# Clemapfel/kmer_index

Hardware: AMD Instinct MI355X
Metric: M queries/sec, DNA4 k=10 exact-match batch search, 1e8-bp text (higher is better)
Workload: dtype u32/u64

## Files before the change

kmer_index_amd/csrc/kmx_capi.hip:

```cpp
#include <hip/hip_runtime.h>

#include <algorithm>
#include <atomic>
#include <cstddef>
#include <cstdio>
#include <cstdlib>
#include <cstring>
#include <functional>
#include <memory>
#include <mutex>
#include <string>
#include <system_error>
#include <thread>
#include <utility>
#include <vector>

#include "kmx_approx.h"
#include "kmx_host.h"
#include "kmx_kernels.h"
#include "kmx_vote.h"

namespace {

thread_local std::string g_err;
// ... 305 lines not shown

void release_idle(ResultPool& pool)
{
    std::vector<kmx_result*> idle;
    { std::lock_guard<std::mutex> lock(pool.mu); idle.swap(pool.idle); }
    for (kmx_result* r : idle) { r->release(); delete r; }
}

kmx_result* take_result(kmx_index* ix)
{
    kmx_result* r = nullptr;
    {
        std::lock_guard<std::mutex> lock(ix->pool->mu);
        if (!ix->pool->idle.empty()) { r = ix->pool->idle.back(); ix->pool->idle.pop_back(); }
    }
    if (!r) r = new kmx_result();
    r->pool = ix->pool;
    return r;
}

template <typename F>
void timed(kmx_index* ix, int id, hipStream_t s, F&& launch)
{
    if (!ix->stats.enabled) { launch(); return; }
    std::lock_guard<std::mutex> lock(ix->stats.mu);
    hipEvent_t a = ix->stats.get(), b = ix->stats.get();
    (void)hipEventRecord(a, s);
    launch();
    (void)hipEventRecord(b, s);
    ix->stats.pending.push_back({id, a, b});
}

template <typename T>
kmx_status upload(kmx_index* ix, const T* host, size_t count, const T** dev_out)
{
    void* p = nullptr;
    size_t bytes = std::max<size_t>(count * sizeof(T), 16) + 16;
    HIP_TRY(hipMalloc(&p, bytes));
    ix->allocs.push_back(p);
    ix->device_bytes += bytes;
    if (count) HIP_TRY(hipMemcpy(p, host, count * sizeof(T), hipMemcpyHostToDevice));
    *dev_out = static_cast<const T*>(p);
    return KMX_OK;
}

struct DeviceScratch {
    std::vector<void*> ptrs;
    ~DeviceScratch() { for (void* p : ptrs) (void)hipFree(p); }
    template <typename T> hipError_t get(T** out, size_t count)
    {
        void* p = nullptr;
        hipError_t e = hipMalloc(&p, count * sizeof(T) + 64);
        if (e == hipSuccess) { ptrs.push_back(p); *out = static_cast<T*>(p); }
        return e;
    }
};

kmx_status check_device()
{
    int count = 0;
    hipError_t e = hipGetDeviceCount(&count);
    if (e != hipSuccess || count <= 0)
        return fail(KMX_ERR_NO_DEVICE, "no HIP device visible: the kmx engine has no CPU search path");
    return KMX_OK;
}

}

static uint32_t cell_shift_for(uint32_t table_kind, uint64_t n_keys, uint64_t npos, uint64_t region, const kmx_options& o)
{
    if (table_kind != KMX_TABLE_DENSE || o.no_aligned_copy || region > npos) return 0;
    if (const char* e = getenv("KMX_CELLS")) { if (!atoi(e)) return 0; }
    const double c = double(npos) / double(n_keys);
    uint32_t shift = c <= 3.5 ? 3u : c <= 10.5 ? 4u : c <= 24.0 ? 5u : 0u;
    if (const char* e = getenv("KMX_CELL_SHIFT")) { const int v = atoi(e); if (v >= 3 && v <= 5) shift = uint32_t(v); }
    if (!shift) return 0;
    if ((n_keys << shift) > 8 * npos) return 0;
    return shift;
}
static inline uint64_t up32_elems(uint64_t v) { return (v + 31) & ~uint64_t(31); }

static hipError_t publish_headers(kmx_index* ix)
{
    hipError_t e = hipMemcpy(ix->d_index, &ix->h_header, sizeof(KmxIndexDev), hipMemcpyHostToDevice);
    if (e == hipSuccess && ix->d_index_fast) {
        KmxIndexDev hf = ix->h_header;
        if (ix->d_plan_fast) hf.plan = ix->d_plan_fast;
        e = hipMemcpy(ix->d_index_fast, &hf, sizeof hf, hipMemcpyHostToDevice);
    }
    return e;
}
static inline const KmxIndexDev* header_for(const kmx_index* ix, uint32_t flags)
{
    static const bool ref_plan_only = getenv("KMX_REFERENCE_PLAN") != nullptr;
    return ((flags & (KMX_SEARCH_KEEP_MASKS | KMX_SEARCH_REFERENCE_PLAN)) || !ix->d_index_fast || ref_plan_only) ? ix->d_index : ix->d_index_fast;
}

static kmx_status install_images_impl(std::vector<kmx::ElemImage>& images, const uint8_t* tail_kmax, uint64_t n, uint32_t sigma,
                                 uint32_t range, int device, const kmx_options& o, kmx_index** out, void* prebuilt_arena,
                                 uint64_t prebuilt_arena_elems = 0)
{
    auto* ix = new kmx_index();
    ix->device = device;
    ix->n = n;
    ix->sigma = sigma;
    ix->range = range;
    const uint32_t n_ks = uint32_t(images.size());
    uint32_t kmax = 0;
    for (auto& im : images) { ix->ks.push_back(im.k); kmax = std::max(kmax, im.k); }
    kmx_status st = KMX_OK;
    auto bail = [&](kmx_status s) { std::string keep = g_err; kmx_index_free(ix); g_err = keep; return s; };
    for (auto& im : images) {
        if (im.d_offs_prebuilt) ix->allocs.push_back(const_cast<uint32_t*>(im.d_offs_prebuilt));
        if (im.d_atab_prebuilt) ix->allocs.push_back(const_cast<uint32_t*>(im.d_atab_prebuilt));
        if (im.d_ukeys_prebuilt) ix->allocs.push_back(const_cast<uint64_t*>(im.d_ukeys_prebuilt));
        if (im.d_slots_prebuilt) ix->allocs.push_back(const_cast<KmxSlot*>(im.d_slots_prebuilt));
    }

    KmxIndexDev h{};
    h.n = n; h.sigma = sigma; h.n_ks = n_ks; h.kmax = kmax; h.range = range;
    for (uint32_t j = 0; j < 64; ++j) {
        unsigned __int128 v = 1;
        for (uint32_t t = 0; t < j; ++t) { v *= sigma; if (v > ~uint64_t(0)) { v = ~uint64_t(0); break; } }
        h.pw[j] = uint64_t(v);
    }
    uint64_t arena_elems = 0;
    for (auto& im : images) {
        if (!im.region) im.region = im.npos;
        if (im.region > im.npos) arena_elems = (arena_elems + 31) & ~uint64_t(31);
        arena_elems += im.region;
    }
    std::vector<uint32_t> cell_shift(n_ks, 0);
    std::vector<uint64_t> cell_base(n_ks, 0);
    for (uint32_t i = 0; i < n_ks; ++i) {
        const auto& im = images[i];
        cell_shift[i] = cell_shift_for(im.table_kind, im.n_keys, im.npos, im.region, o);
        if (cell_shift[i] && (up32_elems(arena_elems) + (im.n_keys << cell_shift[i]) + 65536) * 4 >= (uint64_t(1) << 32)) cell_shift[i] = 0;
        if (!cell_shift[i]) continue;
        arena_elems = up32_elems(arena_elems);
        cell_base[i] = arena_elems;
        arena_elems += im.n_keys << cell_shift[i];
    }
    if (prebuilt_arena && prebuilt_arena_elems < arena_elems) {
        fail(KMX_ERR_INVALID_ARGUMENT, "internal: the prebuilt arena is smaller than the index layout");
        return bail(KMX_ERR_INVALID_ARGUMENT);
    }
    {
        void* p = prebuilt_arena;
        if (!p) {
            hipError_t e = hipMalloc(&p, arena_elems * 4 + KMX_ARENA_PAD);
            if (e != hipSuccess) { fail(KMX_ERR_OUT_OF_MEMORY, std::string("arena: ") + hipGetErrorString(e)); return bail(KMX_ERR_OUT_OF_MEMORY); }
        }
        ix->allocs.push_back(p);
        ix->device_bytes += arena_elems * 4;
        {
            hipError_t e = hipMemset(static_cast<unsigned char*>(p) + arena_elems * 4, 0xFF, KMX_ARENA_PAD);
            if (e != hipSuccess) { fail(KMX_ERR_HIP, std::string("arena padding: ") + hipGetErrorString(e)); return bail(KMX_ERR_HIP); }
        }
        h.arena = static_cast<const uint32_t*>(p);
        ix->d_arena = h.arena;
    }
    h.arena_elems = arena_elems;
    ix->rec32 = (arena_elems + 65536) * 4 < (uint64_t(1) << 32);
    if (const char* f64 = getenv("KMX_FORCE_REC64")) { if (atoi(f64)) ix->rec32 = false; }
    if (const char* fvs = getenv("KMX_FILL_VARIANT")) {
        int e = atoi(fvs);
// ... 2355 lines not shown
```

kmer_index_amd/csrc/kmx_kernels.hip:

```cpp
#include <hip/hip_runtime.h>
#include <stdint.h>

#include <algorithm>
#include <atomic>
#include <type_traits>

#include "kmx_kernels.h"

#define KMX_BLOCK 256
#define KMX_WAVE 64
#define KMX_PSORT_PAIR_CAP 512
#ifndef KMX_PSORT_MULTIWAY_RUNS
#define KMX_PSORT_MULTIWAY_RUNS 4
#endif
#define KMX_PM_WAVE_EMAX (((KMX_PSORT_CAP + (KMX_WAVE - KMX_PSORT_MAX_RUNS / 2) - 1) / (KMX_WAVE - KMX_PSORT_MAX_RUNS / 2)) | 1)
#define KMX_PM_WAVE_PAD (KMX_PSORT_MAX_RUNS + KMX_PM_WAVE_EMAX + 5)
#define KMX_PM_TILE 4096
#define KMX_STAGE_CAP 1024
#define KMX_VGROUP 16
#define KMX_VGROUPS (KMX_WAVE / KMX_VGROUP)
#define KMX_VSLICES (64 / KMX_VGROUP)
#define KMX_VSTAGE (1024 / KMX_VGROUPS)
#define KMX_VCH 8

// ... 328 lines not shown
                            key = extra.src;
                            p1 = (uint64_t(extra_delta) << 32) | extra.cnt | (P - 1 + (rest ? 1 : 0) > 1 ? KMX_P1_MORE : 0);
                            if (!(flags & KMX_SEARCH_KEEP_MASKS) && stitch_goes_big(first.cnt, extra.cnt)) p1 |= KMX_P1_BIG;
                            if (track) {
                                const uint32_t lo = alive ? uint32_t(__ffs(int(alive))) - 1u : 0u, len = uint32_t(__popc(alive));
                                if ((alive >> lo) == (1u << len) - 1u) {
                                    resolved = true;
                                    src = first.src + lo;
                                    cnt = len;
                                }
                            }
                        }
                    }
                }
            }
        } else {
            uint64_t mm = m;
            bool all = true;
            Run r{0, 0}, extra{0, 0};
            uint32_t extra_delta = 0;
            const uint32_t nparts = pe.nparts;
            for (uint32_t j = 0; j < nparts && all && ranks_ok; ++j) {
                const KmxPlanEntry e = load_plan_chain(ix, mm);
                const KmxElemDev* el = &elems_s[e.elem];
                const uint32_t k = el->k;
                mm -= k;
                uint64_t h;
                ranks_ok = rank_hash(qr + mm, k, sigma, h, qend);
                if (!ranks_ok) break;
                r = probe(el, h);
                if (j == 0) {
                    extra = r; extra_delta = uint32_t(mm);
                    track = !(flags & KMX_SEARCH_KEEP_MASKS) && nparts > 1 && sparse_buckets(el) && r.cnt != 0 && r.cnt <= KMX_VRESOLVE;
                    if (track) {
                        alive = 0;
#pragma unroll
                        for (uint32_t i = 0; i < KMX_VRESOLVE; ++i) {
                            const uint32_t a = ar[r.src + (i < r.cnt ? i : 0u)];
                            cand[i] = a - uint32_t(mm);
                            alive |= uint32_t(i < r.cnt && a >= uint32_t(mm)) << i;
                        }
                    }
                } else if (track && r.cnt) {
                    follow(r, uint32_t(mm));
                }
                all = r.cnt != 0;
            }
            if (all && ranks_ok) {
                if (nparts == 1) { kind = KMX_KIND_EXACT; src = r.src; cnt = r.cnt; }
                else {
                    kind = KMX_KIND_STITCH; src = r.src; c0 = r.cnt;
                    key = extra.src;
                    p1 = (uint64_t(extra_delta) << 32) | extra.cnt | (nparts > 2 ? KMX_P1_MORE : 0);
                    if (!(flags & KMX_SEARCH_KEEP_MASKS) && stitch_goes_big(r.cnt, extra.cnt)) p1 |= KMX_P1_BIG;
                    if (track) {
                        uint32_t fmask = 0;
                        for (uint32_t t = 0; t < r.cnt; ++t) {
                            const uint32_t b = ar[r.src + t];
#pragma unroll
                            for (uint32_t i = 0; i < KMX_VRESOLVE; ++i) fmask |= uint32_t(((alive >> i) & 1u) && cand[i] == b) << t;
                        }
                        const uint32_t lo = fmask ? uint32_t(__ffs(int(fmask))) - 1u : 0u, len = uint32_t(__popc(fmask));
                        if ((fmask >> lo) == (1u << len) - 1u) {
                            resolved = true;
                            src = r.src + lo;
                            cnt = len;
                        }
                    }
                }
            }
        }
        if (!ranks_ok) { status = KMX_Q_BAD_RANK; kind = KMX_KIND_NONE; cnt = 0; }
    }
    o.src = src; o.aux = aux; o.key = key; o.p1 = p1; o.cnt = cnt; o.c0 = c0; o.kind = kind; o.status = status; o.resolved = resolved;
}

struct BlockCounters {
    unsigned int n_long, base_long;
    unsigned int n_stitch, n_stitch_tiny, n_stitch_short, n_resolved, n_prefix, n_prefix_big, n_prefix_merge, n_prefix_mid, n_prefix_plain, n_error, n_none, n_more;
    unsigned long long words, pelems, hits;
    unsigned int max_runs;
    unsigned int base_stitch, base_stitch_tiny, base_stitch_short, base_prefix, base_prefix_big;
    unsigned long long base_words;
    unsigned int max_fan_exp;
    unsigned int small_keys;
};

template <bool SMALL>
__device__ __forceinline__ bool hash16(const u32x4_a1& w, uint32_t len, uint32_t sigma, uint64_t& h)
{
    uint64_t lo = uint64_t(w[0]) | (uint64_t(w[1]) << 32), hi = uint64_t(w[2]) | (uint64_t(w[3]) << 32);
    {
        const uint32_t sh = (16u - len) * 8u;
        const uint32_t s6 = sh & 63u;
        const uint64_t carry = s6 ? lo >> (64u - s6) : 0;
        const uint64_t hi1 = (hi << s6) | carry, lo1 = lo << s6;
        hi = sh >= 128u ? 0 : sh >= 64u ? lo1 : hi1;
        lo = sh >= 64u ? 0 : lo1;
    }
    const uint32_t wd[4] = {uint32_t(lo), uint32_t(lo >> 32), uint32_t(hi), uint32_t(hi >> 32)};
    uint32_t top = 0;
    if (SMALL) {
        uint32_t acc = 0;
#pragma unroll
        for (uint32_t j = 0; j < 16; ++j) {
            const uint32_t r = (wd[j >> 2] >> (8 * (j & 3))) & 0xFFu;
            top = max(top, r);
            acc = __umul24(acc, sigma) + r;
        }
        h = acc;
    } else {
        uint64_t acc = 0;
#pragma unroll
        for (uint32_t j = 0; j < 16; ++j) {
            const uint32_t r = (wd[j >> 2] >> (8 * (j & 3))) & 0xFFu;
            top = max(top, r);
            acc = acc * sigma + r;
        }
        h = acc;
    }
    return top < sigma;
}
__device__ __forceinline__ const char* probe_first_addr(const KmxElemDev* el, uint64_t h)
{
    if (el->table_kind == KMX_TABLE_DENSE)
        return el->cnt8 ? reinterpret_cast<const char*>(el->cnt8 + (h & ~uint64_t(15)))
                        : reinterpret_cast<const char*>((el->atab ? el->atab : el->offs) + h);
    return reinterpret_cast<const char*>(el->slots + slot_hash_dev(h, el->log2cap));
}
__device__ __forceinline__ Run probe_finish(const KmxElemDev* el, uint64_t h, const u32x4_a1& pr)
{
    Run r{0, 0};
    if (el->table_kind == KMX_TABLE_DENSE) {
        if (el->cnt8) {
            const uint32_t b = uint32_t(h) & 15u;
            const uint32_t wsel = (b >> 2) == 0 ? pr[0] : (b >> 2) == 1 ? pr[1] : (b >> 2) == 2 ? pr[2] : pr[3];
            const uint32_t c = (wsel >> ((b & 3u) * 8u)) & 0xFFu;
            if (c != 255u) { r.src = el->cell_base + (h << el->cell_shift); r.cnt = c; }
            else {
                const KMX_GLOBAL uint32_t* offs = as_global(el->offs);
                const uint32_t a = offs[h], e = offs[h + 1];
                r.src = el->arena_base + a; r.cnt = e - a;
            }
        }
        else if (el->atab) { r.src = el->arena_base + (pr[0] & ~31u); r.cnt = atab_count(pr[0], pr[1]); }
        else { r.src = el->arena_base + pr[0]; r.cnt = pr[1] - pr[0]; }
        return r;
    }
    const KMX_GLOBAL KmxSlot* slots = as_global(el->slots);
    const uint64_t mask = (uint64_t(1) << el->log2cap) - 1;
    uint64_t s = slot_hash_dev(h, el->log2cap);
    uint64_t key = uint64_t(pr[0]) | (uint64_t(pr[1]) << 32);
    uint32_t off = pr[2], c = pr[3];
    while (c != 0 && key != h) {
        s = (s + 1) & mask;
        const u64x2 raw = *(const KMX_GLOBAL u64x2*)(slots + s);
        key = raw.x; off = uint32_t(raw.y); c = uint32_t(raw.y >> 32);
    }
    if (c) { r.src = el->arena_base + off; r.cnt = c; }
    return r;
}

#define KMX_PLAN_LDS 256

#ifndef KMX_LOOKUP_OCC
#define KMX_LOOKUP_OCC 4
#endif
template <int ITEMS, bool PAIRS>
__global__ __launch_bounds__(KMX_BLOCK, PAIRS ? KMX_LOOKUP_OCC : (ITEMS > 4 ? 4 : 5)) void k_lookup(const KmxIndexDev* __restrict__ ix,
                                                      const uint8_t* __restrict__ qranks,
                                                      const uint64_t* __restrict__ qoff, uint64_t nq,
                                                      QueryDesc d, unsigned long long* __restrict__ ctr,
                                                      uint64_t* __restrict__ block_hits, uint32_t flags)
{
    __shared__ BlockCounters bc;
    __shared__ KmxElemDev elems_s[KMX_MAX_KS];
    __shared__ uint32_t plan_s[KMX_PLAN_LDS];
    static_assert(KMX_PLAN_LDS == KMX_BLOCK, "one planner entry per thread");
    if (threadIdx.x == 0) {
        bc.n_long = 0;
        bc.n_stitch = bc.n_stitch_tiny = bc.n_stitch_short = bc.n_resolved = bc.n_prefix = bc.n_prefix_big = bc.n_prefix_merge = bc.n_prefix_mid = bc.n_prefix_plain = bc.n_error = bc.n_none = bc.n_more = 0;
        bc.words = bc.pelems = bc.hits = 0;
        bc.max_runs = 0;
        unsigned int j = 0;
        while (j < 63 && ix->pw[j + 1] <= KMX_SUBK_FANOUT_LIMIT) ++j;
        bc.max_fan_exp = j;
        unsigned int small = ix->sigma < (1u << 24) ? 1u : 0u;
        for (uint32_t e = 0; e < ix->n_ks; ++e) {
            const uint64_t nk = ix->elems[e].n_keys;
            if (nk > (uint64_t(1) << 32) || nk / ix->sigma > (uint64_t(1) << 24)) small = 0;
        }
        bc.small_keys = small;
    }
    {
        const uint32_t n_words = ix->n_ks * uint32_t(sizeof(KmxElemDev) / 8);
        const uint64_t* __restrict__ srcw = reinterpret_cast<const uint64_t*>(ix->elems);
        uint64_t* dstw = reinterpret_cast<uint64_t*>(elems_s);
        for (uint32_t i = threadIdx.x; i < n_words; i += KMX_BLOCK) dstw[i] = srcw[i];
        plan_s[threadIdx.x] = threadIdx.x < ix->range ? ((const KMX_GLOBAL uint32_t*)ix->plan)[threadIdx.x] : 0u;
    }
    const uint8_t* __restrict__ qend = qranks + qoff[nq];
    __syncthreads();

    uint8_t kinds[ITEMS];
    unsigned int locs[ITEMS];
    unsigned long long locw[ITEMS];
    bool done[ITEMS];
    uint64_t my_hits = 0;
    const uint32_t sigma = ix->sigma, range = ix->range;
    const bool small_keys = __builtin_amdgcn_readfirstlane(int(bc.small_keys)) != 0;
    const uint8_t* __restrict__ dummy = reinterpret_cast<const uint8_t*>(ix);

    unsigned int my_resolved = 0, my_err = 0, my_none = 0;
    auto emit = [&](int it, uint64_t q, uint8_t kind, uint8_t status, uint64_t src, uint64_t aux, uint64_t key, uint64_t p1, uint32_t cnt,
                    uint32_t c0, bool resolved) {
        unsigned int loc = 0;
        unsigned long long loc_words = 0;
        if (kind == KMX_KIND_STITCH && !resolved) {
            const uint32_t pc = uint32_t(p1);
            if (min(c0, pc) <= KMX_VTINY && max(c0, pc) <= 2 * KMX_VTINY) {
                loc = atomicAdd(&bc.n_stitch_tiny, 1u) | 0x80000000u;
            } else if (!(p1 & (KMX_P1_MORE | KMX_P1_BIG)) && min(c0, pc) <= KMX_VSHORT && max(c0, pc) <= KMX_VSTAGE) {
                loc = atomicAdd(&bc.n_stitch_short, 1u) | 0x40000000u;
                if (pc < c0) p1 |= KMX_P1_SWAP;
            } else {
                if ((p1 & (KMX_P1_MORE | KMX_P1_BIG)) || stitch_is_wide(p1)) atomicAdd(&bc.n_more, 1u);
                loc = atomicAdd(&bc.n_stitch, 1u);
            }
            loc_words = atomicAdd(&bc.words, (unsigned long long)(uint64_t(c0) / 64 + 1));
        }
        if (kind == KMX_KIND_PREFIX) {
            const uint32_t plen = cnt - uint32_t(__popcll(aux));
            if (c0 < 2 || plen < 2) {
                loc = 0xFFFFFFFFu;
                atomicAdd(&bc.n_prefix_plain, 1u);
            } else if (KMX_PSORT_IS_SMALL(c0, plen)) {
                loc = atomicAdd(&bc.n_prefix, 1u);
                if (KMX_PSORT_IS_MERGE(c0, plen)) atomicAdd(&bc.n_prefix_merge, 1u);
            } else {
                loc = atomicAdd(&bc.n_prefix_big, 1u) | 0x80000000u;
                if (plen <= KMX_PSORT_MID_CAP) atomicAdd(&bc.n_prefix_mid, 1u);
                if (plen > KMX_PSORT_BLOCK_CAP) {
                    atomicAdd(&bc.pelems, (unsigned long long)plen);
                    atomicMax(&bc.max_runs, (plen + KMX_PSORT_BLOCK_CAP - 1) / KMX_PSORT_BLOCK_CAP);
                }
            }
        }
        my_resolved += resolved;
        my_err += status != KMX_Q_OK;
        my_none += status == KMX_Q_OK && kind == KMX_KIND_NONE;
        kinds[it] = !resolved ? kind : uint8_t(KMX_KIND_NONE);
        locs[it] = loc;
        locw[it] = loc_words;
        my_hits += cnt;
        d.src[q] = (kind == KMX_KIND_STITCH && !resolved) ? (src | SRC_SLOW) : (kind == KMX_KIND_PREFIX ? (src | SRC_FLAGS) : src);
        d.cnt[q] = cnt;
        d.kind[q] = kind;
        d.status[q] = status;
        if (kind == KMX_KIND_STITCH) {
            if (!resolved) {
                d.c0[q] = c0;
                d.key[q] = key;
                d.p1[q] = p1;
            }
        } else if (kind == KMX_KIND_PREFIX) {
            d.c0[q] = c0;
            d.aux[q] = aux;
            d.key[q] = key;
        }
    };

    uint64_t qb[ITEMS];
    uint32_t qm[ITEMS];
    uint32_t praw[ITEMS];
#pragma unroll
    for (int it = 0; it < ITEMS; ++it) {
        const uint64_t q = (uint64_t(blockIdx.x) * ITEMS + it) * KMX_BLOCK + threadIdx.x;
        const uint64_t qq = q < nq ? q : nq - 1;
        qb[it] = qoff[qq];
        const uint64_t mlen = qoff[qq + 1] - qb[it];
        qm[it] = mlen > 0xFFFFFFFFull ? 0xFFFFFFFFu : uint32_t(mlen);
        kinds[it] = KMX_KIND_NONE;
        locs[it] = 0;
        locw[it] = 0;
    }
#pragma unroll
    for (int it = 0; it < ITEMS; ++it)
        praw[it] = plan_effective(((const KMX_GLOBAL uint32_t*)ix->plan)[min(qm[it], range - 1)]);

    {
        uint32_t eab[ITEMS];
        bool two[ITEMS];
        u32x4_a1 wa[ITEMS], wb[ITEMS];
        unsigned int n_none = 0, n_err = 0;
#pragma unroll
        for (int it = 0; it < ITEMS; ++it) {
            const uint64_t q = (uint64_t(blockIdx.x) * ITEMS + it) * KMX_BLOCK + threadIdx.x;
            const uint32_t m = qm[it], scheme = praw[it] & 0xFF, e = (praw[it] >> 8) & 0xFF;
            const uint32_t kb = elems_s[e].k;
            const bool live = q < nq && m > 0 && m < range;
            const bool one = live && scheme == KMX_SCHEME_SINGLE && kb == m && m <= 16 && qranks + qb[it] + 16 <= qend;
            bool t = false;
            uint32_t ea = e, off = 0;
            if (PAIRS && live && !one && m < KMX_PLAN_LDS) {
                if (scheme == KMX_SCHEME_SINGLE) {
                    const uint32_t rest = m < 2 * kb ? m - kb : 0u;
                    t = m > kb && m <= 2 * kb && kb <= 16 && (rest == 0 || kb - rest <= bc.max_fan_exp);
                    off = m - kb;
                } else if (scheme == KMX_SCHEME_MULTI && ((praw[it] >> 16) & KMX_PLAN_NPARTS_MASK) == 2 && m > kb) {
                    const uint32_t p2 = plan_s[m - kb];
                    ea = (p2 >> 8) & 0xFF;
                    const uint32_t ka = elems_s[ea].k;
                    t = (p2 & 0xFF) != KMX_SCHEME_NONE && ka + kb == m && ka <= 16 && kb <= 16;
                    off = m - kb;
                }
                t = t && qranks + qb[it] + off + 16 <= qend;
            }
            done[it] = one || t;
            two[it] = t;
            eab[it] = ea | (e << 8) | (off << 16);
            wa[it] = *reinterpret_cast<const u32x4_a1*>(done[it] ? qranks + qb[it] : dummy);
            if (PAIRS) wb[it] = *reinterpret_cast<const u32x4_a1*>(t ? qranks + qb[it] + off : dummy);
        }
        uint64_t ha[ITEMS], hb[ITEMS];
        bool oka[ITEMS], okb[ITEMS];
        u32x4_a1 pa[ITEMS], pb[ITEMS];
#pragma unroll
        for (int it = 0; it < ITEMS; ++it) {
            const KmxElemDev* ela = &elems_s[eab[it] & 0xFF];
            const KmxElemDev* elb = &elems_s[(eab[it] >> 8) & 0xFF];
            okb[it] = true; hb[it] = 0;
            if (small_keys) {
                oka[it] = hash16<true>(wa[it], done[it] ? ela->k : 0u, sigma, ha[it]);
                if (PAIRS) okb[it] = hash16<true>(wb[it], two[it] ? elb->k : 0u, sigma, hb[it]);
            } else {
                oka[it] = hash16<false>(wa[it], done[it] ? ela->k : 0u, sigma, ha[it]);
                if (PAIRS) okb[it] = hash16<false>(wb[it], two[it] ? elb->k : 0u, sigma, hb[it]);
            }
            pa[it] = *(const KMX_GLOBAL u32x4_a1*)((done[it] && oka[it]) ? probe_first_addr(ela, ha[it]) : reinterpret_cast<const char*>(dummy));
            if (PAIRS) pb[it] = *(const KMX_GLOBAL u32x4_a1*)((two[it] && okb[it]) ? probe_first_addr(elb, hb[it]) : reinterpret_cast<const char*>(dummy));
        }
        struct Pend {
            bool two, tiny, first_is_short;
            uint8_t kind, status;
            uint64_t src, key, p1;
            uint32_t c0, off, pc;
            u32x4 s0, s1, l0, l1, l2, l3;
        };
        const KMX_GLOBAL uint32_t* ar = as_global(ix->arena);
        auto stage1 = [&](int it) -> Pend {
            Pend P{};
            P.two = false; P.tiny = false; P.first_is_short = true; P.kind = KMX_KIND_NONE; P.status = KMX_Q_OK; P.src = P.key = P.p1 = 0; P.c0 = P.off = P.pc = 0;
            const uint64_t q = (uint64_t(blockIdx.x) * ITEMS + it) * KMX_BLOCK + threadIdx.x;
            Run ra{0, 0}, rb{0, 0};
            if (done[it]) {
                const KmxElemDev* ela = &elems_s[eab[it] & 0xFF];
                if (oka[it]) ra = probe_finish(ela, ha[it], pa[it]);
                if (!PAIRS || !two[it]) {
                    const uint8_t status = oka[it] ? KMX_Q_OK : KMX_Q_BAD_RANK;
                    n_err += status != KMX_Q_OK;
                    n_none += status == KMX_Q_OK && !ra.cnt;
                    d.src[q] = ra.src;
                    d.cnt[q] = ra.cnt;
                    d.kind[q] = ra.cnt ? KMX_KIND_EXACT : KMX_KIND_NONE;
                    d.status[q] = status;
                    my_hits += ra.cnt;
                } else {
                    const KmxElemDev* elb = &elems_s[(eab[it] >> 8) & 0xFF];
                    const uint32_t off = eab[it] >> 16;
                    const bool multi = (praw[it] & 0xFF) == KMX_SCHEME_MULTI;
                    if (okb[it]) rb = probe_finish(elb, hb[it], pb[it]);
                    const bool bad = multi ? (!okb[it] || (rb.cnt != 0 && !oka[it])) : (!oka[it] || (ra.cnt != 0 && !okb[it]));
                    P.two = true;
                    if (bad) {
                        P.status = KMX_Q_BAD_RANK;
                    } else if (ra.cnt != 0 && rb.cnt != 0) {
                        P.kind = KMX_KIND_STITCH; P.src = ra.src; P.c0 = ra.cnt; P.key = rb.src; P.off = off; P.pc = rb.cnt;
                        P.p1 = (uint64_t(off) << 32) | rb.cnt;
                        if (!(flags & KMX_SEARCH_KEEP_MASKS) && stitch_goes_big(ra.cnt, rb.cnt)) P.p1 |= KMX_P1_BIG;
                        P.tiny = !(flags & KMX_SEARCH_KEEP_MASKS) && min(ra.cnt, rb.cnt) <= KMX_VTINY && max(ra.cnt, rb.cnt) <= 2 * KMX_VTINY;
                        P.first_is_short = ra.cnt <= rb.cnt;
                    }
                }
            }
            static_assert(KMX_VTINY == 8, "two 16-byte loads for the shorter bucket, four for the longer");
            if (!PAIRS) return P;
            const uint64_t sa = !P.tiny ? 0 : P.first_is_short ? ra.src : rb.src, la = !P.tiny ? 0 : P.first_is_short ? rb.src : ra.src;
            P.s0 = *reinterpret_cast<const KMX_GLOBAL u32x4_a4*>(ar + sa); P.s1 = *reinterpret_cast<const KMX_GLOBAL u32x4_a4*>(ar + sa + 4);
            P.l0 = *reinterpret_cast<const KMX_GLOBAL u32x4_a4*>(ar + la); P.l1 = *reinterpret_cast<const KMX_GLOBAL u32x4_a4*>(ar + la + 4);
            P.l2 = *reinterpret_cast<const KMX_GLOBAL u32x4_a4*>(ar + la + 8); P.l3 = *reinterpret_cast<const KMX_GLOBAL u32x4_a4*>(ar + la + 12);
// ... 1226 lines not shown
    d.p1[q] = p1 & ~KMX_P1_MORE;
}

__global__ __launch_bounds__(KMX_BLOCK) void k_validate_more(const KmxIndexDev* __restrict__ ix,
                                                             const uint32_t* __restrict__ arena,
                                                             const uint8_t* __restrict__ qranks,
                                                             const uint64_t* __restrict__ qoff, QueryDesc d,
                                                             uint64_t n_stitch, uint64_t* __restrict__ mask_words)
{
    const uint32_t lane = lane_id();
    const uint32_t g = lane / KMX_VGROUP, gl = lane % KMX_VGROUP;
    const uint64_t wave = (uint64_t(blockIdx.x) * KMX_BLOCK + threadIdx.x) / KMX_WAVE;
    const uint64_t n_waves = uint64_t(gridDim.x) * (KMX_BLOCK / KMX_WAVE);
    for (uint64_t i0 = wave * KMX_VGROUPS; i0 < n_stitch; i0 += n_waves * KMX_VGROUPS) {
        const uint64_t i = i0 + g;
        const bool have = i < n_stitch;
        const uint32_t q = have ? d.stitch_list[i] : 0u;
        const uint64_t p1 = have ? d.p1[q] : 0;
        const uint32_t tentative = have ? d.cnt[q] : 0u;
        const bool more = !(p1 & KMX_P1_BIG) && (p1 & KMX_P1_MORE) != 0 && tentative != 0;
        const bool big = more && tentative > KMX_VMORE_WAVE;
        const bool active = more && !big;
        uint32_t rounds = active ? tentative : 0u;
#pragma unroll
        for (int e = 1; e < KMX_VGROUPS; ++e) rounds = max(rounds, uint32_t(__shfl_xor(int(rounds), e * KMX_VGROUP)));
        rounds = uint32_t(__builtin_amdgcn_readfirstlane(int(rounds)));
        if (rounds == 0) continue;
        const uint64_t wbase = active ? d.aux[q] : 0;
        uint32_t* __restrict__ hits = d.stitch_hits + wbase * 64;
        uint32_t kept = 0;
        for (uint32_t t = 0; t < rounds; ++t) {
            if (active && t < tentative) {
                const uint32_t p = hits[t];
                const bool good = stitch_parts_hold(ix, arena, qranks, qoff, q, p, gl);
                const uint32_t verdicts = uint32_t(__ballot(good) >> (KMX_VGROUP * g)) & 0xFFFFu;
                if (verdicts == 0xFFFFu) {
                    if (gl == 0 && kept != t) hits[kept] = p;
                    ++kept;
                } else if (gl == 0) {
                    const uint64_t src = d.src[q] & ~SRC_FLAGS;
                    const uint64_t idx = lower_bound_dev<uint32_t>(arena + src, d.c0[q], p);
                    mask_words[wbase + (idx >> 6)] &= ~(uint64_t(1) << (idx & 63));
                }
            }
        }
        if (active && gl == 0) d.cnt[q] = kept;
    }
}

#ifndef KMX_VWAVE_OCC
#define KMX_VWAVE_OCC 4
#endif
__global__ __launch_bounds__(KMX_BLOCK, KMX_VWAVE_OCC) void k_validate_wave(const KmxIndexDev* __restrict__ ix,
                                                             const uint32_t* __restrict__ arena,
                                                             const uint8_t* __restrict__ qranks,
                                                             const uint64_t* __restrict__ qoff, QueryDesc d,
                                                             uint64_t n_stitch, uint64_t* __restrict__ mask_words)
{
    __shared__ uint32_t stage[KMX_BLOCK / KMX_WAVE][KMX_BIG_STAGE];
    const uint32_t lane = lane_id();
    const uint64_t wave = (uint64_t(blockIdx.x) * KMX_BLOCK + threadIdx.x) / KMX_WAVE;
    const uint64_t n_waves = uint64_t(gridDim.x) * (KMX_BLOCK / KMX_WAVE);
    for (uint64_t i0 = wave * KMX_VWAVE_SCAN; i0 < n_stitch; i0 += n_waves * KMX_VWAVE_SCAN) {
        const uint64_t i = i0 + lane;
        const bool have = lane < KMX_VWAVE_SCAN && i < n_stitch;
        const uint32_t q = have ? d.stitch_list[i] : 0u;
        const uint64_t p1 = have ? d.p1[q] : 0;
        const uint32_t tentative = have ? d.cnt[q] : 0u;
        const bool whole = (p1 & KMX_P1_BIG) != 0;
        const bool longlist = !whole && (p1 & KMX_P1_MORE) != 0 && tentative > KMX_VMORE_WAVE;
        uint64_t todo = __ballot(whole || longlist);
        while (todo) {
            const int l = __ffsll((unsigned long long)todo) - 1;
            todo &= todo - 1;
            const uint32_t ql = uint32_t(__shfl(int(q), l));
            if (__shfl(int(whole), l)) validate_big_wave(ix, arena, qranks, qoff, d, ql, stage[threadIdx.x / KMX_WAVE]);
            else validate_more_wave(ix, arena, qranks, qoff, d, ql, uint32_t(__shfl(int(tentative), l)), mask_words);
        }
    }
}

#define KMX_SCAN_ITEMS 16
#define KMX_SCAN_TILE (KMX_BLOCK * KMX_SCAN_ITEMS)

__device__ __forceinline__ uint64_t block_exclusive_scan_u64(uint64_t v, uint64_t* total_out)
{
    __shared__ uint64_t wave_sum[KMX_BLOCK / KMX_WAVE];
    const uint32_t lane = lane_id(), w = threadIdx.x / KMX_WAVE;
    uint64_t inc = v;
    for (int off = 1; off < KMX_WAVE; off <<= 1) {
        uint64_t t = __shfl_up(inc, off);
        if (lane >= uint32_t(off)) inc += t;
    }
    if (lane == KMX_WAVE - 1) wave_sum[w] = inc;
    __syncthreads();
    uint64_t carry = 0, total = 0;
    for (uint32_t i = 0; i < KMX_BLOCK / KMX_WAVE; ++i) {
        uint64_t s = wave_sum[i];
        if (i < w) carry += s;
        total += s;
    }
    __syncthreads();
    if (total_out) *total_out = total;
    return carry + inc - v;
}

__device__ __forceinline__ uint32_t stitch_n_extra(const KmxIndexDev* __restrict__ ix, uint64_t m)
{
    const KmxPlanEntry pe = load_plan(ix, m);
    if (pe.scheme != KMX_SCHEME_SINGLE) return pe.nparts - 1u;
    const uint32_t k = ix->elems[pe.elem].k;
    return uint32_t(m / k) - 1u + ((m % k) ? 1u : 0u);
}

#define KMX_SMALL_XFLAG (1ull << 63)
#define KMX_SMALL_SPIN_LIMIT (1u << 20)
__global__ __launch_bounds__(KMX_BLOCK) void k_small(const KmxIndexDev* __restrict__ ix, const uint32_t* __restrict__ arena,
                                                     unsigned char* __restrict__ mailbox, KmxSmallLayout L, KmxSmallArgs args,
                                                     uint32_t nq_total, unsigned long long* __restrict__ xchg, uint32_t flags)
{
    const uint32_t blk = blockIdx.x, qb = blk * KMX_SMALL_NQ;
    const uint32_t nq = args.nq[blk], n_letters = args.n_letters[blk];
    const unsigned char* __restrict__ in_area = mailbox + size_t(blk) * KMX_SMALL_IN_BYTES;
    constexpr uint32_t NW = KMX_BLOCK / KMX_WAVE;
    static_assert(NW * KMX_SMALL_WCAP == KMX_SMALL_SORT, "the waves share the sort buffer of the workgroup");
    __shared__ __attribute__((aligned(16))) unsigned char s_in[KMX_SMALL_IN_BYTES + 16];
    __shared__ KmxElemDev elems_s[KMX_MAX_KS];
    __shared__ uint64_t s_src[KMX_SMALL_NQ], s_aux[KMX_SMALL_NQ];
    __shared__ uint32_t s_cnt[KMX_SMALL_NQ], s_c0[KMX_SMALL_NQ], s_off[KMX_SMALL_NQ + 1];
    __shared__ uint8_t s_kind[KMX_SMALL_NQ], s_status[KMX_SMALL_NQ];
    __shared__ uint64_t s_words[KMX_SMALL_WORDS];
    __shared__ __attribute__((aligned(16))) uint32_t s_sort[KMX_SMALL_SORT];
    __shared__ uint16_t s_wslow[KMX_SMALL_WSLOW], s_bslow[KMX_SMALL_BSLOW];
    __shared__ uint32_t s_n_wslow, s_n_bslow, s_n_words, s_bad, s_valid, s_n_stitch, s_n_prefix, s_n_error, s_n_none;
    const uint32_t tid = threadIdx.x, lane = lane_id(), wv = threadIdx.x / KMX_WAVE;
    KmxSmallHeader* __restrict__ hdr = reinterpret_cast<KmxSmallHeader*>(mailbox + L.off_header) + blk;
    auto decline = [&] {
        if (threadIdx.x == 0) {
            hdr->fallback = 1;
            if (xchg) __hip_atomic_store((KMX_GLOBAL unsigned long long*)xchg + blk, KMX_SMALL_XFLAG, __ATOMIC_RELAXED, __HIP_MEMORY_SCOPE_AGENT);
        }
    };
    auto wsync = [] {
        __builtin_amdgcn_fence(__ATOMIC_RELEASE, "wavefront");
        __builtin_amdgcn_wave_barrier();
        __builtin_amdgcn_fence(__ATOMIC_ACQUIRE, "wavefront");
    };

    {
        const uint32_t in_bytes = (nq + 1) * 8 + n_letters;
        const uint4* __restrict__ src4 = reinterpret_cast<const uint4*>(in_area);
        uint4* dst4 = reinterpret_cast<uint4*>(s_in);
        for (uint32_t i = tid; i < (in_bytes + 15) / 16; i += KMX_BLOCK) dst4[i] = src4[i];
        const uint32_t n_words = ix->n_ks * uint32_t(sizeof(KmxElemDev) / 8);
        const uint64_t* __restrict__ srcw = reinterpret_cast<const uint64_t*>(ix->elems);
        uint64_t* dstw = reinterpret_cast<uint64_t*>(elems_s);
        for (uint32_t i = tid; i < n_words; i += KMX_BLOCK) dstw[i] = srcw[i];
        if (tid == 0) { s_n_wslow = s_n_bslow = s_n_words = s_bad = s_n_stitch = s_n_prefix = s_n_error = s_n_none = 0; }
    }
    __syncthreads();
    const uint64_t* s_qoff = reinterpret_cast<const uint64_t*>(s_in);
    const uint8_t* s_qr = s_in + (nq + 1) * 8;
    const uint8_t* s_qend = s_qr + n_letters;

    {
        LookupOut lo;
// ... 199 lines not shown
        if (s_kind[q] == KMX_KIND_STITCH) {
            const uint32_t c0 = s_c0[q], wbase = uint32_t(s_aux[q]);
            for (uint32_t c = t; c < c0; c += T) {
                const uint64_t w = s_words[wbase + c / 64];
                if ((w >> (c & 63)) & 1u) {
                    uint32_t rank = uint32_t(__popcll(w & ((uint64_t(1) << (c & 63)) - 1)));
                    for (uint32_t j = 0; j < c / 64; ++j) rank += uint32_t(__popcll(s_words[wbase + j]));
                    out[s_off[q] + rank] = arena[src + c];
                }
            }
        } else {
            const uint32_t len = s_cnt[q] - uint32_t(__popcll(s_aux[q]));
            uint32_t n2 = 2;
            while (n2 < len) n2 <<= 1;
            sync();
            for (uint32_t i = t; i < n2; i += T) sbuf[i] = i < len ? arena[src + i] : 0xFFFFFFFFu;
            sync();
            bitonic_lds(sbuf, n2, t, T, sync);
            for (uint32_t i = t; i < len; i += T) out[s_off[q] + i] = sbuf[i];
        }
    };
    __syncthreads();
    for (uint32_t si = wv; si < n_wslow; si += NW) emit(s_wslow[si], lane, KMX_WAVE, s_sort + wv * KMX_SMALL_WCAP, wsync);
    __syncthreads();
    for (uint32_t si = 0; si < n_bslow; ++si) emit(bslow_at(si), tid, KMX_BLOCK, s_sort, [] { __syncthreads(); });
    if (tid == 0) {
        hdr->nq = nq;
        hdr->n_hits = total;
        hdr->n_mask_words = s_n_words;
        hdr->n_stitch = s_n_stitch; hdr->n_prefix = s_n_prefix; hdr->n_error = s_n_error; hdr->n_none = s_n_none;
        hdr->fallback = 0;
    }
}

void launch_small(hipStream_t s, const KmxIndexDev* ix, const uint32_t* arena, unsigned char* mailbox, const KmxSmallLayout& layout, uint32_t n_blocks,
                  const KmxSmallArgs& args, uint32_t nq_total, unsigned long long* xchg, uint32_t flags)
{
    hipLaunchKernelGGL(k_small, dim3(n_blocks), dim3(KMX_BLOCK), 0, s, ix, arena, mailbox, layout, args, nq_total, xchg, flags);
}

__global__ __launch_bounds__(KMX_BLOCK) void k_scan_reduce(const uint32_t* __restrict__ in, uint64_t n,
                                                           uint64_t* __restrict__ bsum)
{
    const uint64_t base = uint64_t(blockIdx.x) * KMX_SCAN_TILE;
    uint64_t s = 0;
#pragma unroll
    for (int j = 0; j < KMX_SCAN_ITEMS; ++j) {
        uint64_t i = base + uint64_t(j) * KMX_BLOCK + threadIdx.x;
        if (i < n) s += in[i];
    }
    uint64_t total;
    block_exclusive_scan_u64(s, &total);
    if (threadIdx.x == 0) bsum[blockIdx.x] = total;
}

__global__ __launch_bounds__(KMX_BLOCK) void k_scan_spine(uint64_t* __restrict__ bsum, uint64_t nb,
                                                          unsigned long long* __restrict__ total_out)
{
    uint64_t running = 0;
    for (uint64_t base = 0; base < nb; base += KMX_BLOCK) {
        uint64_t i = base + threadIdx.x;
        uint64_t v = i < nb ? bsum[i] : 0;
        uint64_t total;
        uint64_t ex = block_exclusive_scan_u64(v, &total);
        if (i < nb) bsum[i] = running + ex;
        running += total;
    }
    if (threadIdx.x == 0) *total_out = running;
}

template <bool TILES, int SPINE>
__global__ __launch_bounds__(KMX_BLOCK) void k_scan_down(const uint32_t* __restrict__ in, uint64_t n,
                                                         const uint64_t* __restrict__ bsum,
                                                         uint64_t* __restrict__ out, uint64_t tile,
                                                         uint64_t n_tiles_cap, uint32_t* __restrict__ tile_q,
                                                         unsigned long long* __restrict__ total_out, uint64_t n_fine,
                                                         CounterPub pub, uint32_t fine_per_tile)
{
    static_assert(KMX_SCAN_TILE % (KMX_BLOCK * 8) == 0 && KMX_SCAN_TILE % (KMX_BLOCK * 4) == 0, "a scan tile is a whole number of lookup blocks");
    constexpr int ROWS = KMX_SCAN_ITEMS / 4;
    __shared__ uint64_t wave_sum[ROWS][KMX_BLOCK / KMX_WAVE];
    const uint32_t lane = lane_id(), w = threadIdx.x / KMX_WAVE;
    const uint64_t block_base = uint64_t(blockIdx.x) * KMX_SCAN_TILE;
    uint32_t v[ROWS][4];
    uint64_t inc[ROWS];
#pragma unroll
    for (int r = 0; r < ROWS; ++r) {
        const uint64_t i = block_base + uint64_t(r) * (KMX_BLOCK * 4) + uint64_t(threadIdx.x) * 4;
        if (i + 3 < n) {
            const uint4 t = *reinterpret_cast<const uint4*>(in + i);
            v[r][0] = t.x; v[r][1] = t.y; v[r][2] = t.z; v[r][3] = t.w;
        } else {
#pragma unroll
            for (int j = 0; j < 4; ++j) v[r][j] = i + j < n ? in[i + j] : 0u;
        }
        inc[r] = uint64_t(v[r][0]) + v[r][1] + v[r][2] + v[r][3];
    }
    uint64_t own[ROWS];
#pragma unroll
    for (int r = 0; r < ROWS; ++r) own[r] = inc[r];
    for (int off = 1; off < KMX_WAVE; off <<= 1) {
#pragma unroll
        for (int r = 0; r < ROWS; ++r) {
            const uint64_t t = __shfl_up(inc[r], off);
            if (lane >= uint32_t(off)) inc[r] += t;
        }
    }
    if (lane == KMX_WAVE - 1) {
#pragma unroll
        for (int r = 0; r < ROWS; ++r) wave_sum[r][w] = inc[r];
    }
    __syncthreads();
    uint64_t row_base;
    if constexpr (SPINE != 0) {
        __shared__ uint64_t part[KMX_BLOCK / KMX_WAVE];
        const uint64_t mine = SPINE == 2 ? uint64_t(blockIdx.x) * fine_per_tile : uint64_t(blockIdx.x);
        uint64_t acc = 0;
        for (uint64_t i = threadIdx.x; i < mine; i += KMX_BLOCK) acc += bsum[i];
        for (int off = 32; off > 0; off >>= 1) acc += __shfl_xor(acc, off);
        if (lane == 0) part[w] = acc;
        __syncthreads();
        row_base = 0;
#pragma unroll
        for (uint32_t i = 0; i < KMX_BLOCK / KMX_WAVE; ++i) row_base += part[i];
        if (blockIdx.x + 1 == gridDim.x && threadIdx.x == 0) {
            uint64_t own = 0;
            if constexpr (SPINE == 2) { for (uint64_t i = mine; i < n_fine; ++i) own += bsum[i]; }
            else own = bsum[blockIdx.x];
            *total_out = row_base + own;
            if (pub.host) {
#pragma unroll
                for (int c = 0; c < KMX_CTR_COUNT; ++c) {
                    pub.host[c] = c == KMX_CTR_TOTAL_HITS ? row_base + own : pub.cur[c];
                    pub.next[c] = 0;
                }
            }
        }
    } else {
        row_base = bsum[blockIdx.x];
    }
#pragma unroll
    for (int r = 0; r < ROWS; ++r) {
        uint64_t carry = 0, total = 0;
#pragma unroll
        for (uint32_t i = 0; i < KMX_BLOCK / KMX_WAVE; ++i) {
            const uint64_t sw = wave_sum[r][i];
            if (i < w) carry += sw;
            total += sw;
        }
        uint64_t ex = row_base + carry + inc[r] - own[r];
        row_base += total;
        const uint64_t i0 = block_base + uint64_t(r) * (KMX_BLOCK * 4) + uint64_t(threadIdx.x) * 4;
        uint64_t o[4];
#pragma unroll
        for (int j = 0; j < 4; ++j) {
            const uint64_t i = i0 + j;
            o[j] = ex;
            if constexpr (TILES) {
                if (i < n && v[r][j]) {
                    uint64_t t = (ex + tile - 1) / tile;
                    const uint64_t t_end = (ex + v[r][j] - 1) / tile;
                    for (; t <= t_end && t <= n_tiles_cap; ++t) tile_q[t] = uint32_t(i);
                }
            }
            ex += v[r][j];
            if (i + 1 == n) {
                out[n] = ex;
                if constexpr (TILES) {
                    for (uint64_t t = (ex + tile - 1) / tile; t <= n_tiles_cap && t <= (ex + tile - 1) / tile + 1; ++t) tile_q[t] = uint32_t(n - 1);
                }
            }
        }
        if (i0 + 3 < n) {
            typedef uint64_t u64x2s __attribute__((ext_vector_type(2)));
            u64x2s a, c;
            a[0] = o[0]; a[1] = o[1]; c[0] = o[2]; c[1] = o[3];
            *reinterpret_cast<u64x2s*>(out + i0) = a;
            *reinterpret_cast<u64x2s*>(out + i0 + 2) = c;
        } else {
#pragma unroll
            for (int j = 0; j < 4; ++j)
                if (i0 + j < n) out[i0 + j] = o[j];
        }
    }
    if (n == 0 && blockIdx.x == 0 && threadIdx.x == 0) out[0] = 0;
}

__global__ __launch_bounds__(KMX_BLOCK) void k_partition(const uint64_t* __restrict__ off, uint64_t nq,
                                                         uint64_t tile, uint64_t n_tiles,
                                                         uint32_t* __restrict__ tile_q)
{
    const uint64_t t = uint64_t(blockIdx.x) * KMX_BLOCK + threadIdx.x;
    if (t > n_tiles) return;
    const uint64_t x = t * tile;
    uint64_t ub = upper_bound_dev<uint64_t>(off, nq + 1, x);
    uint64_t qi = ub ? ub - 1 : 0;
    if (qi > nq - 1) qi = nq - 1;
    tile_q[t] = uint32_t(qi);
}


template <typename rec_t>
struct RecTraits {
    static constexpr rec_t SLOW = rec_t(1) << (sizeof(rec_t) * 8 - 1);
};

template <int E, bool NT, typename rec_t>
__global__ __launch_bounds__(KMX_BLOCK, (E <= 12 ? 8 : 6)) void k_fill(const KmxIndexDev* __restrict__ ix,
                                                    const uint32_t* __restrict__ arena,
                                                    const uint64_t* __restrict__ hit_off,
                                                    const uint32_t* __restrict__ tile_q,
                                                    const unsigned long long* __restrict__ total_dev,
                                                    QueryDesc d, uint32_t* __restrict__ out)
{
    constexpr int TILE = KMX_BLOCK * E;
    const uint64_t total = *total_dev;
// ... 2307 lines not shown
```

kmer_index_amd/csrc/kmx_types.h:

```cpp
#pragma once
#include <stdint.h>
#include "../../include/kmx.h"

#define KMX_MAX_LEVELS 3
#define KMX_DEFAULT_PREFIX_LEVELS 2

struct KmxSlot {
    uint64_t key;
    uint32_t off;
    uint32_t cnt;
};

struct KmxElemDev {
    uint32_t k;
    uint32_t table_kind;
    uint32_t log2cap;
    uint32_t n_ukeys;
    uint64_t n_keys;
    uint64_t arena_base;
    uint64_t npos;
    const uint32_t* offs;
    const KmxSlot* slots;
    const uint64_t* ukeys;
    const uint32_t* atab;
    uint64_t region;
    const uint32_t* dir;
    uint32_t dir_shift;
    uint32_t n_dir;
    const uint8_t* cnt8;
    uint64_t cell_base;
    uint32_t cell_shift;
    uint32_t n_levels;
    uint64_t lvl_offs_at[KMX_MAX_LEVELS];
    uint64_t lvl_base[KMX_MAX_LEVELS];
};

enum { KMX_SCHEME_NONE = 0, KMX_SCHEME_SINGLE = 1, KMX_SCHEME_MULTI = 2, KMX_SCHEME_REPLANNED = 3 };
#define KMX_PLAN_ALT_SHIFT 11
#define KMX_PLAN_NPARTS_MASK ((1u << KMX_PLAN_ALT_SHIFT) - 1u)
struct KmxPlanEntry {
    uint8_t scheme;
    uint8_t elem;
    uint16_t nparts;
};

struct KmxIndexDev {
    uint64_t n;
    uint32_t sigma;
    uint32_t n_ks;
    uint32_t kmax;
    uint32_t range;
    const uint32_t* arena;
    const uint8_t* tail;
    const KmxPlanEntry* plan;
    uint64_t arena_elems;
    unsigned long long* dbg;
    uint64_t pw[64];
    KmxElemDev elems[KMX_MAX_KS];
};

#define KMX_PSORT_IS_SMALL(runs, len) ((len) <= KMX_PSORT_CAP)
#ifndef KMX_PMERGE_MIN_AVG
#define KMX_PMERGE_MIN_AVG 8
#endif
#define KMX_PSORT_IS_MERGE(runs, len)                                                                                   \
    ((len) <= KMX_PSORT_CAP && (runs) >= 2 && (runs) <= KMX_PSORT_MAX_RUNS && !((runs) <= KMX_PMERGE_REG_RUNS && (len) <= KMX_PMERGE_REG_LEN) && \
     (len) >= KMX_PMERGE_MIN_AVG * (runs))
#ifndef KMX_PMERGE_REG_RUNS
#define KMX_PMERGE_REG_RUNS 4
#endif
#ifndef KMX_PMERGE_REG_LEN
#define KMX_PMERGE_REG_LEN 512
#endif
#define KMX_VRESOLVE 4
#define KMX_ARENA_PAD (4096 * 4 + 1024)
#define KMX_VTINY 8
#define KMX_VSHORT 16
#define KMX_PSORT_MAX_RUNS 32
#define KMX_PSORT_CAP 2048
#define KMX_PSORT_BLOCK_CAP 32768
#define KMX_PSORT_MID_CAP 8192

#define KMX_SMALL_NQ 256
#define KMX_SMALL_BLOCKS 32
struct KmxSmallArgs {
    uint16_t nq[KMX_SMALL_BLOCKS];
    uint16_t n_letters[KMX_SMALL_BLOCKS];
};
#define KMX_SMALL_IN_BYTES 8192
#define KMX_SMALL_WCAP 1024
#define KMX_SMALL_WSLOW 32
#define KMX_SMALL_SORT 4096
#define KMX_SMALL_BSLOW 8
#define KMX_SMALL_WORDS (KMX_SMALL_WSLOW * (KMX_SMALL_WCAP / 64 + 1) + KMX_SMALL_BSLOW * (KMX_SMALL_SORT / 64 + 1))
#define KMX_SMALL_POS 49152
struct KmxSmallHeader {
    uint32_t fallback;
    uint32_t nq;
    uint64_t n_hits, n_mask_words;
    uint32_t n_stitch, n_prefix, n_error, n_none;
    uint32_t pad[6];
};
struct KmxSmallLayout {
    uint32_t blocks, off_header, off_hitoff, off_csrc, off_mbase, off_ccnt, off_status, off_kinds, off_words, off_pos, bytes, pad;
};
static inline KmxSmallLayout kmx_small_layout(uint32_t blocks)
{
    KmxSmallLayout L;
    const uint32_t nq = blocks * KMX_SMALL_NQ;
    L.blocks = blocks;
    L.off_header = blocks * KMX_SMALL_IN_BYTES;
    L.off_hitoff = L.off_header + blocks * 64;
    L.off_csrc = L.off_hitoff + (nq + 2) * 8;
    L.off_mbase = L.off_csrc + nq * 8;
    L.off_ccnt = L.off_mbase + nq * 8;
    L.off_status = L.off_ccnt + nq * 4;
    L.off_kinds = L.off_status + nq;
    L.off_words = L.off_kinds + nq;
    L.off_pos = L.off_words + blocks * KMX_SMALL_WORDS * 8;
    L.bytes = L.off_pos + blocks * KMX_SMALL_POS * 4;
    L.pad = 0;
    return L;
}

enum {
    KMX_CTR_STITCH = 1,
    KMX_CTR_PREFIX = 2,
    KMX_CTR_ERROR = 3,
    KMX_CTR_MASK_WORDS = 4,
    KMX_CTR_PREFIX_ELEMS = 5,
    KMX_CTR_MAX_RUNS = 6,
    KMX_CTR_TOTAL_HITS = 7,
    KMX_CTR_NONE = 8,
    KMX_CTR_PREFIX_TOTAL = 9,
    KMX_CTR_STITCH_MORE = 10,
    KMX_CTR_PREFIX_BIG = 11,
    KMX_CTR_STITCH_TINY = 12,
    KMX_CTR_STITCH_RESOLVED = 13,
    KMX_CTR_PREFIX_MERGE = 14,
    KMX_CTR_PREFIX_MID = 15,
// ... 13 lines not shown
```

Measured before the change: 7031.

## Precompute lookup header flags on host and vectorize scan spine prefix

```diff
diff --git a/kmer_index_amd/csrc/kmx_capi.hip b/kmer_index_amd/csrc/kmx_capi.hip
--- a/kmer_index_amd/csrc/kmx_capi.hip
+++ b/kmer_index_amd/csrc/kmx_capi.hip
@@ -411,6 +411,18 @@
 
 static hipError_t publish_headers(kmx_index* ix)
 {
+    {
+        KmxIndexDev& h = ix->h_header;
+        uint32_t j = 0;
+        while (j < 63 && h.pw[j + 1] <= KMX_SUBK_FANOUT_LIMIT) ++j;
+        h.max_fan_exp = j;
+        uint32_t small = h.sigma < (1u << 24) ? 1u : 0u;
+        for (uint32_t el = 0; el < h.n_ks; ++el) {
+            const uint64_t nk = h.elems[el].n_keys;
+            if (nk > (uint64_t(1) << 32) || nk / h.sigma > (uint64_t(1) << 24)) small = 0;
+        }
+        h.small_keys = small;
+    }
     hipError_t e = hipMemcpy(ix->d_index, &ix->h_header, sizeof(KmxIndexDev), hipMemcpyHostToDevice);
     if (e == hipSuccess && ix->d_index_fast) {
         KmxIndexDev hf = ix->h_header;
diff --git a/kmer_index_amd/csrc/kmx_kernels.hip b/kmer_index_amd/csrc/kmx_kernels.hip
--- a/kmer_index_amd/csrc/kmx_kernels.hip
+++ b/kmer_index_amd/csrc/kmx_kernels.hip
@@ -434,8 +434,6 @@
     unsigned int max_runs;
     unsigned int base_stitch, base_stitch_tiny, base_stitch_short, base_prefix, base_prefix_big;
     unsigned long long base_words;
-    unsigned int max_fan_exp;
-    unsigned int small_keys;
 };
 
 template <bool SMALL>
@@ -534,15 +532,6 @@
         bc.n_stitch = bc.n_stitch_tiny = bc.n_stitch_short = bc.n_resolved = bc.n_prefix = bc.n_prefix_big = bc.n_prefix_merge = bc.n_prefix_mid = bc.n_prefix_plain = bc.n_error = bc.n_none = bc.n_more = 0;
         bc.words = bc.pelems = bc.hits = 0;
         bc.max_runs = 0;
-        unsigned int j = 0;
-        while (j < 63 && ix->pw[j + 1] <= KMX_SUBK_FANOUT_LIMIT) ++j;
-        bc.max_fan_exp = j;
-        unsigned int small = ix->sigma < (1u << 24) ? 1u : 0u;
-        for (uint32_t e = 0; e < ix->n_ks; ++e) {
-            const uint64_t nk = ix->elems[e].n_keys;
-            if (nk > (uint64_t(1) << 32) || nk / ix->sigma > (uint64_t(1) << 24)) small = 0;
-        }
-        bc.small_keys = small;
     }
     {
         const uint32_t n_words = ix->n_ks * uint32_t(sizeof(KmxElemDev) / 8);
@@ -560,7 +549,8 @@
     bool done[ITEMS];
     uint64_t my_hits = 0;
     const uint32_t sigma = ix->sigma, range = ix->range;
-    const bool small_keys = __builtin_amdgcn_readfirstlane(int(bc.small_keys)) != 0;
+    const bool small_keys = ix->small_keys != 0;
+    const uint32_t max_fan_exp = ix->max_fan_exp;
     const uint8_t* __restrict__ dummy = reinterpret_cast<const uint8_t*>(ix);
 
     unsigned int my_resolved = 0, my_err = 0, my_none = 0;
@@ -637,8 +627,10 @@
         locw[it] = 0;
     }
 #pragma unroll
-    for (int it = 0; it < ITEMS; ++it)
-        praw[it] = plan_effective(((const KMX_GLOBAL uint32_t*)ix->plan)[min(qm[it], range - 1)]);
+    for (int it = 0; it < ITEMS; ++it) {
+        const uint32_t pi = min(qm[it], range - 1);
+        praw[it] = plan_effective(pi < KMX_PLAN_LDS ? plan_s[pi] : ((const KMX_GLOBAL uint32_t*)ix->plan)[pi]);
+    }
 
     {
         uint32_t eab[ITEMS];
@@ -657,7 +649,7 @@
             if (PAIRS && live && !one && m < KMX_PLAN_LDS) {
                 if (scheme == KMX_SCHEME_SINGLE) {
                     const uint32_t rest = m < 2 * kb ? m - kb : 0u;
-                    t = m > kb && m <= 2 * kb && kb <= 16 && (rest == 0 || kb - rest <= bc.max_fan_exp);
+                    t = m > kb && m <= 2 * kb && kb <= 16 && (rest == 0 || kb - rest <= max_fan_exp);
                     off = m - kb;
                 } else if (scheme == KMX_SCHEME_MULTI && ((praw[it] >> 16) & KMX_PLAN_NPARTS_MASK) == 2 && m > kb) {
                     const uint32_t p2 = plan_s[m - kb];
@@ -2050,6 +2042,7 @@
 
 #define KMX_SCAN_ITEMS 16
 #define KMX_SCAN_TILE (KMX_BLOCK * KMX_SCAN_ITEMS)
+#define KMX_SPINE_BATCH 8
 
 __device__ __forceinline__ uint64_t block_exclusive_scan_u64(uint64_t v, uint64_t* total_out)
 {
@@ -2415,20 +2408,53 @@
     __shared__ uint64_t wave_sum[ROWS][KMX_BLOCK / KMX_WAVE];
     const uint32_t lane = lane_id(), w = threadIdx.x / KMX_WAVE;
     const uint64_t block_base = uint64_t(blockIdx.x) * KMX_SCAN_TILE;
+    typedef uint64_t u64x2s __attribute__((ext_vector_type(2)));
+    const uint64_t spine_pairs = SPINE == 2 ? (uint64_t(blockIdx.x) * fine_per_tile) >> 1 : 0;
+    u64x2s sp[KMX_SPINE_BATCH];
+    auto spine_load = [&](uint64_t base) {
+#pragma unroll
+        for (int j = 0; j < KMX_SPINE_BATCH; ++j) {
+            const uint64_t p = base + uint64_t(j) * KMX_BLOCK + threadIdx.x;
+            sp[j] = u64x2s{0, 0};
+            if (p < spine_pairs) sp[j] = reinterpret_cast<const u64x2s*>(bsum)[p];
+        }
+    };
+    if constexpr (SPINE == 2) spine_load(0);
     uint32_t v[ROWS][4];
     uint64_t inc[ROWS];
-#pragma unroll
-    for (int r = 0; r < ROWS; ++r) {
-        const uint64_t i = block_base + uint64_t(r) * (KMX_BLOCK * 4) + uint64_t(threadIdx.x) * 4;
-        if (i + 3 < n) {
-            const uint4 t = *reinterpret_cast<const uint4*>(in + i);
+    if (block_base + KMX_SCAN_TILE <= n) {
+#pragma unroll
+        for (int r = 0; r < ROWS; ++r) {
+            const uint4 t = *reinterpret_cast<const uint4*>(in + block_base + uint64_t(r) * (KMX_BLOCK * 4) + uint64_t(threadIdx.x) * 4);
             v[r][0] = t.x; v[r][1] = t.y; v[r][2] = t.z; v[r][3] = t.w;
-        } else {
-#pragma unroll
-            for (int j = 0; j < 4; ++j) v[r][j] = i + j < n ? in[i + j] : 0u;
-        }
-        inc[r] = uint64_t(v[r][0]) + v[r][1] + v[r][2] + v[r][3];
-    }
+        }
+    } else {
+#pragma unroll
+        for (int r = 0; r < ROWS; ++r) {
+            const uint64_t i = block_base + uint64_t(r) * (KMX_BLOCK * 4) + uint64_t(threadIdx.x) * 4;
+            if (i + 3 < n) {
+                const uint4 t = *reinterpret_cast<const uint4*>(in + i);
+                v[r][0] = t.x; v[r][1] = t.y; v[r][2] = t.z; v[r][3] = t.w;
+            } else {
+#pragma unroll
+                for (int j = 0; j < 4; ++j) v[r][j] = i + j < n ? in[i + j] : 0u;
+            }
+        }
+    }
+    uint64_t spine_acc = 0;
+    if constexpr (SPINE == 2) {
+        for (uint64_t base = 0;;) {
+#pragma unroll
+            for (int j = 0; j < KMX_SPINE_BATCH; ++j) spine_acc += sp[j][0] + sp[j][1];
+            base += uint64_t(KMX_BLOCK) * KMX_SPINE_BATCH;
+            if (base >= spine_pairs) break;
+            spine_load(base);
+        }
+        const uint64_t mine = uint64_t(blockIdx.x) * fine_per_tile;
+        if ((mine & 1) && threadIdx.x == 0) spine_acc += bsum[mine - 1];
+    }
+#pragma unroll
+    for (int r = 0; r < ROWS; ++r) inc[r] = uint64_t(v[r][0]) + v[r][1] + v[r][2] + v[r][3];
     uint64_t own[ROWS];
 #pragma unroll
     for (int r = 0; r < ROWS; ++r) own[r] = inc[r];
@@ -2443,28 +2469,35 @@
 #pragma unroll
         for (int r = 0; r < ROWS; ++r) wave_sum[r][w] = inc[r];
     }
+    __shared__ uint64_t part[KMX_BLOCK / KMX_WAVE];
+    if constexpr (SPINE == 2) {
+        for (int off = 32; off > 0; off >>= 1) spine_acc += __shfl_xor(spine_acc, off);
+        if (lane == 0) part[w] = spine_acc;
+    }
     __syncthreads();
     uint64_t row_base;
     if constexpr (SPINE != 0) {
-        __shared__ uint64_t part[KMX_BLOCK / KMX_WAVE];
-        const uint64_t mine = SPINE == 2 ? uint64_t(blockIdx.x) * fine_per_tile : uint64_t(blockIdx.x);
-        uint64_t acc = 0;
-        for (uint64_t i = threadIdx.x; i < mine; i += KMX_BLOCK) acc += bsum[i];
-        for (int off = 32; off > 0; off >>= 1) acc += __shfl_xor(acc, off);
-        if (lane == 0) part[w] = acc;
-        __syncthreads();
+        if constexpr (SPINE == 1) {
+            uint64_t acc = 0;
+            for (uint64_t i = threadIdx.x; i < uint64_t(blockIdx.x); i += KMX_BLOCK) acc += bsum[i];
+            for (int off = 32; off > 0; off >>= 1) acc += __shfl_xor(acc, off);
+            if (lane == 0) part[w] = acc;
+            __syncthreads();
+        }
         row_base = 0;
 #pragma unroll
         for (uint32_t i = 0; i < KMX_BLOCK / KMX_WAVE; ++i) row_base += part[i];
         if (blockIdx.x + 1 == gridDim.x && threadIdx.x == 0) {
-            uint64_t own = 0;
-            if constexpr (SPINE == 2) { for (uint64_t i = mine; i < n_fine; ++i) own += bsum[i]; }
-            else own = bsum[blockIdx.x];
-            *total_out = row_base + own;
+            uint64_t own_total = 0;
+#pragma unroll
+            for (int r = 0; r < ROWS; ++r)
+#pragma unroll
+                for (uint32_t i = 0; i < KMX_BLOCK / KMX_WAVE; ++i) own_total += wave_sum[r][i];
+            *total_out = row_base + own_total;
             if (pub.host) {
 #pragma unroll
                 for (int c = 0; c < KMX_CTR_COUNT; ++c) {
-                    pub.host[c] = c == KMX_CTR_TOTAL_HITS ? row_base + own : pub.cur[c];
+                    pub.host[c] = c == KMX_CTR_TOTAL_HITS ? row_base + own_total : pub.cur[c];
                     pub.next[c] = 0;
                 }
             }
diff --git a/kmer_index_amd/csrc/kmx_types.h b/kmer_index_amd/csrc/kmx_types.h
--- a/kmer_index_amd/csrc/kmx_types.h
+++ b/kmer_index_amd/csrc/kmx_types.h
@@ -56,6 +56,8 @@
     uint64_t arena_elems;
     unsigned long long* dbg;
     uint64_t pw[64];
+    uint32_t max_fan_exp;
+    uint32_t small_keys;
     KmxElemDev elems[KMX_MAX_KS];
 };
 
```

Result: no change. 7099 (median of 6 runs) (+1.0%).
